# aelmiger/LINE-MOD-Pipeline

Hardware: AMD Instinct MI355X
Metric: detections/sec (higher is better)
Workload: dtype u8

## Files before the change

line-mod-pipeline_amd/build.py:

```python
import os
import subprocess
import sys

HERE = os.path.dirname(os.path.abspath(__file__))
CSRC = os.path.join(HERE, "csrc")
LIB_DIR = os.path.join(HERE, "lib")
LIB = os.path.join(LIB_DIR, "liblinemod_hip.so")
HIP_SOURCES = ["lm_k_preprocess.hip", "lm_k_mask.hip", "lm_k_scan.hip", "lm_k_refine.hip", "lm_k_post.hip", "lm_k_icp.hip", "lm_k_verify.hip", "lm_k_gen.hip", "lm_k_eval.hip",
               "lm_detector.hip", "lm_detector_upload.hip", "lm_detector_post.hip", "lm_detector_gather.hip", "lm_detector_io.hip", "lm_detector_debug.hip", "lm_detector_icp.hip", "lm_detector_gen.hip", "lm_detector_eval.hip", "lm_comm.hip"]
CXX_SOURCES = ["lm_host.cpp", "lm_extract.cpp", "lm_yaml.cpp"]
HEADERS = ["lm_common.h", "lm_kernels.h", "lm_dev.h", "lm_dev_color.h", "lm_dev_depth.h", "lm_dev_memories.h", "lm_detector_impl.h", "lm_host.h", "lm_extract.h", "lm_median25.h", "lm_yaml.h", "lm_comm.h",
           os.path.join("..", "..", "include", "linemod_hip.h")]
FLAGS = ["-O3", "-std=c++17", "-fPIC", "-ffp-contract=off", "-Wall", "-Wno-unused-function", "-Wno-unused-value"]
ARCH = "gfx950"


def _stale(target, deps):
    if not os.path.exists(target):
        return True
    t = os.path.getmtime(target)
    return any(os.path.exists(d) and os.path.getmtime(d) > t for d in deps)


def build(force=False, verbose=False):
    hipcc = os.environ.get("HIPCC", "/opt/rocm/bin/hipcc")
    os.makedirs(LIB_DIR, exist_ok=True)
    obj_dir = os.path.join(HERE, "build")
    os.makedirs(obj_dir, exist_ok=True)
    headers = [os.path.join(CSRC, h) for h in HEADERS]
    for h in headers:
        if not os.path.exists(h):
            raise FileNotFoundError("header missing from the checkout: " + h)
    objs, cmds = [], []
    for src in HIP_SOURCES + CXX_SOURCES:
        sp = os.path.join(CSRC, src)
        if not os.path.exists(sp):
            raise FileNotFoundError("source file missing from the checkout: " + sp)
        obj = os.path.join(obj_dir, src + ".o")
        objs.append(obj)
        if force or _stale(obj, [sp] + headers + [os.path.abspath(__file__)]):
            cmd = [hipcc] + FLAGS
            if src.endswith(".hip"):
                cmd += ["--offload-arch=" + ARCH]
            else:
                cmd += ["-x", "c++"]
            cmds.append(cmd + ["-c", sp, "-o", obj])
    if cmds:
        from concurrent.futures import ThreadPoolExecutor
        try:
            ncpu = len(os.sched_getaffinity(0))
        except AttributeError:
            ncpu = os.cpu_count() or 1
        jobs = max(1, min(len(cmds), int(os.environ.get("LM_BUILD_JOBS", "0")) or min(ncpu, 8)))

        def run(cmd):
            if verbose:
                print(" ".join(cmd), file=sys.stderr)
            subprocess.check_call(cmd)
        with ThreadPoolExecutor(max_workers=jobs) as ex:
            list(ex.map(run, cmds))
    if force or _stale(LIB, objs):
        cmd = [hipcc, "-shared", "-fPIC", "--offload-arch=" + ARCH, "-o", LIB] + objs + ["-lz", "-ldl"]
        if verbose:
            print(" ".join(cmd), file=sys.stderr)
        subprocess.check_call(cmd)
    return LIB


if __name__ == "__main__":
    print(build(force="--force" in sys.argv, verbose=True))
```

line-mod-pipeline_amd/csrc/lm_detector.hip:

```cpp
#include "lm_detector_impl.h"

namespace lmd {

thread_local std::string g_err;
int fail(int code, const std::string& msg) { g_err = msg; return code; }

bool any_lane_busy(const lm_detector* d) {
    for (const lm_detector::Lane& ln : d->lanes) if (ln.busy) return true;
    return false;
}

void free_device_bank(lm_detector* d) {
    hipFree(d->d_item_t); hipFree(d->d_item_chunk); hipFree(d->d_scan_off); hipFree(d->d_scan_P);
    hipFree(d->d_scan_n); hipFree(d->d_t_global); hipFree(d->d_t_class);
    hipFree(d->d_off1); hipFree(d->d_offn); hipFree(d->d_offs3); d->d_off1 = d->d_offn = d->d_offs3 = nullptr;
    hipFree(d->d_offl); hipFree(d->d_offsl); hipFree(d->d_litem); d->d_offl = d->d_offsl = d->d_litem = nullptr;
    for (auto& it : d->items1) { hipFree(it.d_t); hipFree(it.d_chunk); }
    d->items1.clear();
    d->d_item_t = d->d_item_chunk = d->d_scan_off = nullptr;
    d->d_scan_P = d->d_scan_n = d->d_t_global = d->d_t_class = nullptr;
    for (int l = 0; l < LM_MAX_LEVELS; ++l) {
        hipFree(d->d_ref_meta[l]); hipFree(d->d_ref_feat[l]);
        d->d_ref_meta[l] = nullptr; d->d_ref_feat[l] = nullptr;
    }
}


int ensure_device(lm_detector* d) {
    if (d->dev_ready) {
        HIP_TRY(hipSetDevice(d->cfg.device));
        return LM_OK;
    }
    int ndev = 0;
    hipError_t e = hipGetDeviceCount(&ndev);
    if (e != hipSuccess || ndev <= 0)
        return fail(LM_ERR_NO_DEVICE, "no HIP device available: liblinemod_hip has no CPU fallback");
    if (d->cfg.device < 0 || d->cfg.device >= ndev) return fail(LM_ERR_INVALID, "device ordinal out of range");
    HIP_TRY(hipSetDevice(d->cfg.device));
    d->scanl_lds = lmk_scanl_raise_lds();
    const lm_config& c = d->cfg;
    const int M = c.num_modalities, L = c.pyramid_levels, S = c.frame_slots;
    size_t off = 0;
    d->off_bgr[0] = off; off += (size_t)c.width * c.height * 3;
    d->off_depth = off; off += align_up((size_t)c.width * c.height * 2, 256);
    off = align_up(off, 256);
    for (int l = 1; l < L; ++l) { d->off_bgr[l] = off; off += align_up((size_t)d->lw[l] * d->lh[l] * 3, 256); }
    for (int l = 0; l < L; ++l)
        for (int m = 0; m < M; ++m) { d->off_quant[l][m] = off; off += align_up((size_t)d->lw[l] * d->lh[l], 256); }
    for (int l = 0; l < L; ++l) { d->off_lm[l] = off; off += align_up(d->geom[l].arena_bytes, 256); }
    d->off_cscratch = off; off += align_up(lmk_color_scratch_bytes(c.width, c.height), 256);
    d->off_cscratch1 = off; off += align_up(lmk_color_scratch_bytes(d->lw[L > 1 ? 1 : 0], d->lh[L > 1 ? 1 : 0]), 256);
    d->off_dscratch = off; off += align_up((size_t)c.width * c.height, 256);
    d->cmask_wpr = (c.width + 31) / 32;
    d->off_cmask = off; off += align_up((size_t)d->cmask_wpr * c.height * 4, 256);
    d->match_mask_pitch = align_up((size_t)c.width, 64);
    d->frame_stride = align_up(off, 4096);
    HIP_TRY(hipMalloc(reinterpret_cast<void**>(&d->frame_arena), d->frame_stride * S));
    HIP_TRY(hipMemset(d->frame_arena, 0, d->frame_stride * S));
    off = 0;
    d->off_hdr = off; off += 256;
    d->off_cand = off; off += align_up((size_t)d->max_cand * sizeof(LmCand), 256);
    d->off_keys = off; off += align_up((size_t)d->max_match * 16, 256);
    d->off_out = off; off += align_up((size_t)LM_SORT_CAP * sizeof(LmOutMatch), 256);
    d->aux_stride = align_up(off, 4096);
    HIP_TRY(hipMalloc(reinterpret_cast<void**>(&d->aux_arena), d->aux_stride * S));
    HIP_TRY(hipMemset(d->aux_arena, 0, d->aux_stride * S));
    d->host_stride = align_up(sizeof(LmHostBlock), 256);
    HIP_TRY(hipHostMalloc(reinterpret_cast<void**>(&d->host_blocks), d->host_stride * S, hipHostMallocMapped));
    std::memset(d->host_blocks, 0, d->host_stride * S);
    lm_detector::Lane& l0 = d->lanes[0];
    HIP_TRY(hipMalloc(reinterpret_cast<void**>(&l0.d_raw_thr), 128 * sizeof(int)));
    HIP_TRY(hipHostMalloc(reinterpret_cast<void**>(&l0.h_raw_thr), 128 * sizeof(int)));
    d->plan_stride_cap = std::max(S / 8, 1) + 8;
    const size_t plan_words = 24 * (size_t)d->plan_stride_cap + 16;
    HIP_TRY(hipMalloc(reinterpret_cast<void**>(&d->d_plan), LM_NLANES * plan_words * sizeof(u32)));
    for (int l = 0; l < LM_NLANES; ++l) d->lanes[l].plan = d->d_plan + (size_t)l * plan_words;
    HIP_TRY(hipStreamCreateWithFlags(&l0.stream, hipStreamNonBlocking));
    for (int l = 1; l < LM_NLANES; ++l) HIP_TRY(hipStreamCreateWithFlags(&d->lanes[l].stream, hipStreamNonBlocking));
    for (int k = 0; k < LM_NCOPY; ++k) {
        HIP_TRY(hipStreamCreateWithFlags(&d->copy_stream[k], hipStreamNonBlocking));
        d->up_seq_next[k] = 1; d->up_seq_done[k] = 0;
    }
    for (auto& ev : l0.ev) HIP_TRY(hipEventCreate(&ev));
    l0.created = true;
    d->slots.assign(S, Slot());
    for (Slot& s : d->slots) {
        HIP_TRY(hipEventCreateWithFlags(&s.ev_up, hipEventDisableTiming));
        HIP_TRY(hipEventCreateWithFlags(&s.ev_bgr, hipEventDisableTiming));
    }
    HIP_TRY(hipMalloc(reinterpret_cast<void**>(&d->d_resp_tab), 256 * sizeof(u64) + 256));
    HIP_TRY(hipMalloc(reinterpret_cast<void**>(&d->d_scan_stat), 4096 * sizeof(unsigned long long)));
    HIP_TRY(hipMemset(d->d_scan_stat, 0, 4096 * sizeof(unsigned long long)));
    HIP_TRY(hipMalloc(reinterpret_cast<void**>(&d->d_sim_lut), 256));
    HIP_TRY(hipMalloc(reinterpret_cast<void**>(&d->d_normal_lut), 2 * 8000 + 16));
    HIP_TRY(hipDeviceSynchronize());
    if (const char* ev = getenv("LM_REFINE_STAT")) {
        if (atoi(ev) > 0 && hipMalloc(reinterpret_cast<void**>(&d->d_refine_stat), 8 * sizeof(unsigned long long)) == hipSuccess)
            (void)hipMemset(d->d_refine_stat, 0, 8 * sizeof(unsigned long long));
    }
    d->dev_ready = true;
    d->luts_dirty = true;
    d->bank_dirty = true; d->hulls_dirty = true;
    return LM_OK;
}

int ensure_luts(lm_detector* d) {
    if (!d->luts_dirty) return LM_OK;
    u64 tab[256 + 32];
    u8* miss = reinterpret_cast<u8*>(tab + 256);
    int below4 = 0;
    for (int v = 0; v < 256; ++v) {
        u64 e = 0;
        miss[v] = 0;
        for (int o = 0; o < 8; ++o) {
            u8 r = std::max(d->sim_lut[32 * o + (v & 15)], d->sim_lut[32 * o + 16 + (v >> 4)]);
            e |= (u64)r << (8 * o);
            if (r < 4) { miss[v] |= (u8)(1u << o); below4 = std::max(below4, (int)r); }
        }
        tab[v] = e;
    }
    d->miss_delta = 4 - below4;
    HIP_TRY(hipDeviceSynchronize());
    HIP_TRY(hipMemcpy(d->d_resp_tab, tab, sizeof(tab), hipMemcpyHostToDevice));
    HIP_TRY(hipMemcpy(d->d_sim_lut, d->sim_lut, 256, hipMemcpyHostToDevice));
    {
        u8 both[2 * 8000 + 16] = {};
        std::memcpy(both, d->normal_lut, 8000);
        for (int i = 0; i < 8000; ++i) {
            const u8 v = d->normal_lut[i];
            const unsigned rank = v ? (unsigned)__builtin_ffs((int)v) : 0u;
            both[LMK_NORMAL_CODE_OFFSET + i] = (u8)(rank < 4 ? 8 * rank : (rank < 8 ? 8 * (rank - 4) + 4 : 32u));
        }
        HIP_TRY(hipMemcpy(d->d_normal_lut, both, sizeof(both), hipMemcpyHostToDevice));
    }
    d->luts_dirty = false;
    return LM_OK;
}

int ensure_bank(lm_detector* d) {
    if (!d->bank_dirty) return LM_OK;
    HIP_TRY(hipDeviceSynchronize());
    free_device_bank(d);
    std::string err;
    if (!lmh::build_device_bank(d->bank, d->cfg, d->geom, d->hb, d->scan_list_order, err)) return fail(LM_ERR_INVALID, err);
    int rc;
    if ((rc = upload_vec(&d->d_item_t, d->hb.item_t))) return rc;
    if ((rc = upload_vec(&d->d_item_chunk, d->hb.item_chunk))) return rc;
    if ((rc = upload_vec(&d->d_scan_off, d->hb.scan_off))) return rc;
    if ((rc = upload_vec(&d->d_scan_P, d->hb.scan_P))) return rc;
    if ((rc = upload_vec(&d->d_scan_n, d->hb.scan_n))) return rc;
    if (d->hb.fpad1) {
        if ((rc = upload_vec(&d->d_off1, d->hb.off1))) return rc;
        if ((rc = upload_vec(&d->d_offn, d->hb.offn))) return rc;
        if ((rc = upload_vec(&d->d_offs3, d->hb.offs3))) return rc;
    }
    if (d->hb.lds_ok) {
        if ((rc = upload_vec(&d->d_offl, d->hb.offl))) return rc;
        if ((rc = upload_vec(&d->d_offsl, d->hb.offsl))) return rc;
        if ((rc = upload_vec(&d->d_litem, d->hb.lrec))) return rc;
    }
    if ((rc = upload_vec(&d->d_t_global, d->hb.t_global))) return rc;
    if ((rc = upload_vec(&d->d_t_class, d->hb.t_class))) return rc;
    for (int l = 0; l + 1 < d->cfg.pyramid_levels; ++l) {
        if ((rc = upload_vec(&d->d_ref_meta[l], d->hb.ref_meta[l]))) return rc;
        if ((rc = upload_vec(&d->d_ref_feat[l], d->hb.ref_feat[l]))) return rc;
    }
    d->bank_dirty = false;
    return LM_OK;
}

int check_slots(lm_detector* d, int first, int n) {
    if (first < 0 || n < 0 || first + n > (int)d->slots.size()) return fail(LM_ERR_INVALID, "slot out of range");
    return LM_OK;
}

bool normal_lut_onehot(lm_detector* d) {
    if (d->lut_onehot < 0) {
        d->lut_onehot = 1;
        for (int i = 0; i < 8000; ++i) { const u8 v = d->normal_lut[i]; if (v & (v - 1)) { d->lut_onehot = 0; break; } }
    }
    return d->lut_onehot != 0;
}

void enqueue_depth_pyramid(lm_detector* d, lm_detector::Lane& ln, int first, int n) {
    for (int l = 1; l < d->cfg.pyramid_levels; ++l)
        lmk_nn_half(ln.stream, d->quant(first, l - 1, 1), d->lw[l - 1], d->quant(first, l, 1), d->lw[l], d->lh[l],
                    d->frame_stride, n);
}

int refuse_checked_slots(const lm_detector* d, int first, int n) {
    if (d->cc_inflight && d->cc_pending && first <= d->cc_hi && d->cc_lo < first + n) return fail(LM_ERR_INVALID, "slot is read by a colour check in flight: call lm_color_check_end first");
    if (d->dc_inflight && d->dc_pending && first <= d->dc_hi && d->dc_lo < first + n) return fail(LM_ERR_INVALID, "slot is read by depth counts in flight: call lm_depth_counts_end first");
    const int icp_slot = d->icp_slot.load();
    if (icp_slot >= first && icp_slot < first + n) return fail(LM_ERR_INVALID, "slot is read by an ICP refinement in flight");
    return LM_OK;
}

lmh::ScanInputs scan_inputs(const lm_detector* d, const lm_detector::Lane& ln) {
    const LmLevelGeom& g = d->geom[d->cfg.pyramid_levels - 1];
    lmh::ScanInputs in;
    in.form = d->scan_form; in.M = d->cfg.num_modalities;
    in.nibble = g.nibble != 0; in.planes = g.plane_ori != 0; in.lds_fits = lmh::lds_image_fits(g, in.M);
    in.bank_built = !d->bank_dirty;
    in.scanl_bank = d->hb.lds_ok && d->d_litem; in.scanl_device = d->scanl_lds;
    in.fpad1 = d->hb.fpad1; in.items1_by_L = d->hb.items1_by_L; in.items4 = (long long)d->hb.item_t.size();
    in.frame_stride = d->frame_stride; in.arena_bytes = g.arena_bytes;
    in.threshold = ln.raw_thr_for; in.scan1_min_threshold = d->scan1_min_threshold;
    in.scanl_min_slots = d->scanl_min_slots; in.scanl_R = d->scanl_R;
    return in;
}

void enqueue_lm(lm_detector* d, lm_detector::Lane& ln, int first, int n, int l, int m, u32 planes) {
    hipStream_t st = ln.stream;
    const size_t fs = d->frame_stride;
    const LmLevelGeom& g = d->geom[l];
    const int sp = g.spread_only ? 1 : g.nibble ? 2 : 0;
    u8* dst = d->lm(first, l) + (size_t)m * g.mod_stride;
    if (m == 0 || l == 0)
        lmk_linear_memories(st, d->quant(first, l, m), g.w, 0, sp, g.w, g.h, g.T, d->d_resp_tab, dst, g.ori_stride, fs, fs, n, planes);
    else
        lmk_linear_memories(st, d->quant(first, l - 1, 1), d->lw[l - 1], 1, sp, g.w, g.h, g.T, d->d_resp_tab, dst,
                            g.ori_stride, fs, fs, n, planes);
}

int slot_weight(const lm_detector* d) {
    const long px = (long)d->lw[0] * d->lh[0];
    const int w = d->work_weight_by_pixels ? (int)(px / (640L * 480L)) : 1;
    return w < 1 ? 1 : w;
}

bool any_match_mask(const lm_detector* d, int first, int n) {
    for (int i = first; i < first + n; ++i)
        if (d->slots[i].match_mask_on[0] || d->slots[i].match_mask_on[1] || d->slots[i].rule_on) return true;
    return false;
}

int hsv_bound(double b) { return (int)std::lrint(std::min(256.0, std::max(-1.0, b))); }

int ensure_hsv_div(lm_detector* d) {
    if (d->d_hsv_div) return LM_OK;
    std::vector<int> tab(512, 0);
    for (int i = 1; i < 256; ++i) {
        tab[(size_t)i] = (int)std::lrint((255 << 12) / (1.0 * i));
        tab[256 + (size_t)i] = (int)std::lrint((180 << 12) / (6.0 * i));
    }
    int* p = nullptr;
    HIP_TRY(hipMalloc(reinterpret_cast<void**>(&p), tab.size() * sizeof(int)));
    hipStream_t st = d->lanes[0].stream;
    if (hipMemcpyAsync(p, tab.data(), tab.size() * sizeof(int), hipMemcpyHostToDevice, st) != hipSuccess ||
        hipStreamSynchronize(st) != hipSuccess) {
        (void)hipFree(p);
        return fail(LM_ERR_HIP, "upload of the HSV division tables failed");
    }
    d->d_hsv_div = p;
    return LM_OK;
}

int check_mask_rule(const lm_detector* d, const lm_mask_rule* r, LmRule* out) {
    const lm_config& c = d->cfg;
    if (r->modalities <= 0 || r->modalities >= (1 << c.num_modalities))
        return fail(LM_ERR_INVALID, "mask rule: modalities must name at least one modality the detector has (bit 0 colour, bit 1 depth)");
    if (r->use_depth && c.num_modalities < 2)
        return fail(LM_ERR_INVALID, "mask rule: a depth gate needs the depth frame, which a colour-only detector does not keep on the device");
    if (r->use_depth && (r->zmin < 0 || r->zmax > 65535 || r->zmin > r->zmax))
        return fail(LM_ERR_INVALID, "mask rule: depth gate needs 0 <= zmin <= zmax <= 65535");
    if (r->grow < 0 || r->grow > LM_RULE_MAX_GROW) return fail(LM_ERR_INVALID, "mask rule: grow out of range (0 .. 16)");
    const lm_rect& q = r->rect;
    const bool no_rect = q.width == 0 && q.height == 0;
    if (!no_rect && (q.x < 0 || q.y < 0 || q.width <= 0 || q.height <= 0 || q.x > c.width - q.width || q.y > c.height - q.height))
        return fail(LM_ERR_INVALID, "mask rule: the rectangle must lie inside the frame");
    if (!lmk_mask_rule_fits(c.width)) return fail(LM_ERR_INVALID, "mask rule: frame too wide for the rule kernel");
    LmRule o{};
    o.use_depth = r->use_depth != 0; o.keep_invalid = r->keep_invalid != 0; o.use_hsv = r->use_hsv != 0;
    o.zmin = r->zmin; o.zmax = r->zmax; o.grow = r->grow;
    for (int k = 0; k < 3; ++k) { o.hsv.lo[k] = hsv_bound(r->lower[k]); o.hsv.hi[k] = hsv_bound(r->upper[k]); }
    o.rx = no_rect ? 0 : q.x; o.ry = no_rect ? 0 : q.y; o.rw = no_rect ? c.width : q.width; o.rh = no_rect ? c.height : q.height;
    *out = o;
    return LM_OK;
}

void enqueue_mask_rules(lm_detector* d, lm_detector::Lane& ln, int first, int n) {
    const lm_config& c = d->cfg;
    LmRuleArgs a{};
    a.bgr = d->bgr(0, 0); a.depth = c.num_modalities == 2 ? d->depth(0) : nullptr; a.slot_stride = d->frame_stride;
    a.divtab = d->d_hsv_div; a.w = c.width; a.h = c.height; a.mask_pitch = (u32)d->match_mask_pitch;
    int kinds = 0;
    for (int i = first; i < first + n; ++i) {
        const Slot& s = d->slots[i];
        if (!s.rule_on) continue;
        int k = 0;
        while (k < kinds && std::memcmp(&a.rule[k], &s.rule_dev, sizeof(LmRule)) != 0) ++k;
        if (k == LM_RULE_KINDS) { lmk_mask_rule(ln.stream, a); a.n = 0; kinds = 0; k = 0; }
        if (k == kinds) a.rule[kinds++] = s.rule_dev;
        a.slot[a.n] = (u16)i; a.kind[a.n] = (u8)k; a.plane[a.n] = s.d_rule_mask;
        if (++a.n == LM_MASK_SLOTS) { lmk_mask_rule(ln.stream, a); a.n = 0; kinds = 0; }
    }
    lmk_mask_rule(ln.stream, a);
}

static_assert(LM_MAX_LEVELS <= LM_MASK_LEVELS, "LmMaskArgs holds LM_MASK_LEVELS levels");
void enqueue_match_masks(lm_detector* d, lm_detector::Lane& ln, int first, int n) {
    const lm_config& c = d->cfg;
    LmMaskArgs a{};
    a.frame = d->frame_arena; a.slot_stride = d->frame_stride;
    a.levels = c.pyramid_levels; a.mask_pitch = (u32)d->match_mask_pitch;
    a.vec_rows = 1;
    for (int l = 0; l < c.pyramid_levels; ++l) {
        for (int m = 0; m < c.num_modalities; ++m) a.off_quant[l][m] = (u32)d->off_quant[l][m];
        a.w[l] = (u32)d->lw[l];
        a.vec_begin[l + 1] = a.vec_begin[l] + (u32)((size_t)d->lw[l] * d->lh[l] / 16);
        if (d->lw[l] % 16) a.vec_rows = 0;
    }
    a.vec_depth = a.vec_begin[1];
    for (int i = first; i < first + n; ++i) {
        const Slot& s = d->slots[i];
        if (!s.match_mask_on[0] && !(c.num_modalities == 2 && s.match_mask_on[1])) continue;
        a.slot[a.n] = (u16)i;
        a.cmask[a.n] = s.match_mask_on[0] ? s.d_match_mask : nullptr;
        a.dmask[a.n] = (c.num_modalities == 2 && s.match_mask_on[1]) ? s.d_match_mask + d->match_mask_pitch * c.height : nullptr;
        if (++a.n == LM_MASK_SLOTS) { lmk_match_mask(ln.stream, a); a.n = 0; }
    }
    if (a.n) lmk_match_mask(ln.stream, a);
    a.n = 0;
    for (int i = first; i < first + n; ++i) {
        const Slot& s = d->slots[i];
        if (!s.rule_on) continue;
        a.slot[a.n] = (u16)i;
        a.cmask[a.n] = (s.rule.modalities & 1) ? s.d_rule_mask : nullptr;
        a.dmask[a.n] = (c.num_modalities == 2 && (s.rule.modalities & 2)) ? s.d_rule_mask : nullptr;
        if (++a.n == LM_MASK_SLOTS) { lmk_match_mask(ln.stream, a); a.n = 0; }
    }
    if (a.n) lmk_match_mask(ln.stream, a);
}

void enqueue_preprocess(lm_detector* d, lm_detector::Lane& ln, int first, int n) {
    const lm_config& c = d->cfg;
    const int M = c.num_modalities, L = c.pyramid_levels;
    const lmh::Layout layout = lmh::plan_layout(scan_inputs(d, ln), n);
    for (int i = 0; i < n; ++i) d->slots[first + i].layout = layout;
    const u32 planes = layout == lmh::Layout::Responses ? 0u : d->geom[L - 1].plane_ori | (layout == lmh::Layout::SpreadAndPlanes ? 0x80000000u : 0u);
    const size_t fs = d->frame_stride;
    const int weight = slot_weight(d);
    struct WeightGuard { explicit WeightGuard(int w) { lmk_set_slot_weight(w); } ~WeightGuard() { lmk_set_slot_weight(1); } } weight_guard(weight);
    const int n_eff = n * weight;
    const bool few = n_eff <= d->phase_max_slots;
    bool others_busy = false;
    for (int o = 0; o < LM_NLANES; ++o) others_busy |= (&d->lanes[o] != &ln && d->lanes[o].busy);
    const bool fuse_batch = d->batch_phases == 1 || (d->batch_phases == 2 && !others_busy);
    const bool masked = any_match_mask(d, first, n);
    if (!masked && (few || (fuse_batch && n_eff >= 16)) && L == 2) {
        LmPhaseArgs pa{};
        pa.bgr0 = d->bgr(first, 0); pa.bgr1 = d->bgr(first, 1); pa.depth = M == 2 ? d->depth(first) : nullptr;
        pa.cs0 = d->cscratch(first, 0); pa.cs1 = d->cscratch(first, 1); pa.ds = d->dscratch(first);
        pa.qc0 = d->quant(first, 0, 0); pa.qc1 = d->quant(first, 1, 0); pa.qd0 = M == 2 ? d->quant(first, 0, 1) : nullptr;
        pa.lm_c0 = d->lm(first, 0); pa.lm_c1 = d->lm(first, 1);
        pa.lm_d0 = d->lm(first, 0) + d->geom[0].mod_stride; pa.lm_d1 = d->lm(first, 1) + d->geom[1].mod_stride;
        pa.w = d->lw[0]; pa.h = d->lh[0];
        pa.weak_threshold = c.weak_threshold; pa.dist_thr = c.distance_threshold; pa.diff_thr = c.difference_threshold;
        pa.normal_lut = d->d_normal_lut; pa.resp_tab = d->d_resp_tab; pa.ori_stride1 = d->geom[1].ori_stride; pa.plane_ori1 = planes;
        pa.slot_stride = fs; pa.nslots = n;
        auto mode = [&](int l) { return d->geom[l].spread_only ? 1 : d->geom[l].nibble ? 2 : 0; };
        const bool onehot = M == 2 ? normal_lut_onehot(d) : true;
        if (M <= 2 && d->lw[1] * 2 == d->lw[0] && d->lh[1] * 2 == d->lh[0]) {
            if (few && lmk_phases_supported(pa, d->geom[0].T, d->geom[1].T, mode(0), mode(1), onehot)) {
                lmk_preprocess_phases(ln.stream, pa, d->geom[0].T);
                return;
            }
            if (!few && lmk_batch_phases_supported(pa, d->geom[0].T, d->geom[1].T, mode(0), mode(1), onehot)) {
                lmk_preprocess_batch_phases(ln.stream, pa, d->geom[0].T);
                return;
            }
        }
    }
    const bool blur_pyr = L >= 2 && lmk_blur_pyrdown(ln.stream, d->bgr(first, 0), d->lw[0], d->lh[0], d->cscratch(first, 0), d->bgr(first, 1),
                                                      d->quant(first, 0, 0), fs, n);
    bool grads_done = false;
    if (L == 2 && blur_pyr && d->lw[1] * 2 == d->lw[0] && d->lh[1] * 2 == d->lh[0] && lmk_cgrad_levels_wanted(d->lw[0], d->lh[0], n) &&
        lmk_color_blur(ln.stream, d->bgr(first, 1), d->lw[1], d->lh[1], d->cscratch(first, 1), fs, n)) {
        grads_done = lmk_cgrad_levels(ln.stream, d->cscratch(first, 0), d->lw[0], d->lh[0], d->quant(first, 0, 0), d->cscratch(first, 1), d->lw[1], d->lh[1],
                                      d->quant(first, 1, 0), c.weak_threshold, fs, n);
        if (!grads_done)
            for (int l = 0; l < L; ++l) lmk_color_quantize(ln.stream, d->bgr(first, l), d->lw[l], d->lh[l], c.weak_threshold, d->quant(first, l, 0), nullptr, d->cscratch(first, l), fs, n, true);
        grads_done = true;
    }
    for (int l = 0; l < L; ++l) {
        if (l > 0 && !(l == 1 && blur_pyr)) lmk_pyrdown(ln.stream, d->bgr(first, l - 1), d->lw[l - 1], d->lh[l - 1], d->bgr(first, l), fs, n);
        if (!grads_done)
        lmk_color_quantize(ln.stream, d->bgr(first, l), d->lw[l], d->lh[l], c.weak_threshold, d->quant(first, l, 0),
                           nullptr, d->cscratch(first, l), fs, n, l == 0 && blur_pyr);
        if (M == 2 && l == 0)
            lmk_depth_quantize(ln.stream, d->depth(first), d->lw[0], d->lh[0], c.distance_threshold,
                               c.difference_threshold, d->d_normal_lut, normal_lut_onehot(d), d->quant(first, 0, 1),
                               d->dscratch(first), fs, n);
    }
    if (masked) {
        enqueue_mask_rules(d, ln, first, n);
        enqueue_match_masks(d, ln, first, n);
    }
    if (M == 2 && L > 2) enqueue_depth_pyramid(d, ln, first, n);
    for (int l = 0; l < L; ++l)
        for (int m = 0; m < M; ++m) enqueue_lm(d, ln, first, n, l, m, l == L - 1 ? planes : 0u);
}

void fill_raw_thr(int* tab, float threshold) {
    for (int n = 0; n < 128; ++n) tab[n] = static_cast<int>(2 * n + (threshold / 100.f) * (2 * n) + 0.5f);
}

int item_range(lm_detector* d, int class_idx, ItemRange* r) {
    const int nc = (int)d->bank.classes.size();
    if (class_idx >= nc || class_idx < -1) return fail(LM_ERR_INVALID, "class index out of range");
    if (class_idx < 0) { r->lo = 0; r->n = (int)d->hb.item_t.size(); r->t_lo = 0; r->t_hi = (int)d->hb.t_global.size(); }
    else {
        r->lo = d->hb.class_item_lo[class_idx]; r->n = d->hb.class_item_hi[class_idx] - r->lo;
        r->t_lo = d->hb.class_t_lo[class_idx]; r->t_hi = d->hb.class_t_hi[class_idx];
    }
    return LM_OK;
}

int item_ranges(lm_detector* d, std::vector<int>& classes, std::vector<ItemRange>& out) {
    const int nc = (int)d->bank.classes.size();
    out.clear();
    for (int c : classes) if (c < -1 || c >= nc) return fail(LM_ERR_INVALID, "class index out of range");
    std::sort(classes.begin(), classes.end());
    classes.erase(std::unique(classes.begin(), classes.end()), classes.end());
    if (classes.empty() || classes[0] < 0) {
        if (classes.size() > 1) return fail(LM_ERR_INVALID, "class index -1 (all classes) cannot be combined with others");
        classes.assign(1, -1);
        out.push_back(ItemRange{0, (int)d->hb.item_t.size(), 0, (int)d->hb.t_global.size()});
        return LM_OK;
    }
    for (int c : classes) {
        const int lo = d->hb.class_item_lo[c], hi = d->hb.class_item_hi[c];
        if (!out.empty() && out.back().lo + out.back().n == lo && out.back().t_hi == d->hb.class_t_lo[c]) { out.back().n += hi - lo; out.back().t_hi = d->hb.class_t_hi[c]; }
        else out.push_back(ItemRange{lo, hi - lo, d->hb.class_t_lo[c], d->hb.class_t_hi[c]});
// ... 842 lines not shown
```

line-mod-pipeline_amd/csrc/lm_dev_depth.h:

```cpp
#pragma once
#include "lm_dev.h"
#include "lm_median25.h"

namespace {

#define DT_W 64
#define DT_H 8
#define N_W (DT_W + 4)
#define N_H (DT_H + 4)
#define D_W (DT_W + 14)
#define D_H (DT_H + 14)
#define D_PITCH 80
#define D_LOADS ((D_H * D_W + 255) / 256)

typedef unsigned short us2 __attribute__((ext_vector_type(2)));
#define LM_CE(a, b) { us2 t_ = __builtin_elementwise_min(a, b); b = __builtin_elementwise_max(a, b); a = t_; }

__global__ __launch_bounds__(256) void k_depth_quantize(const u16* __restrict__ depth0, int w, int h, int dist_thr,
                                                         int diff_thr, const u8* __restrict__ lut,
                                                         u8* __restrict__ quant0, size_t slot_stride) {
    __shared__ u16 dt[D_H][D_PITCH];
    __shared__ u8 nt[N_H][N_W + 4];
    const u16* depth = slot_ptr(depth0, slot_stride);
    u8* quant = slot_ptr(quant0, slot_stride);
    const int tid = threadIdx.x;
    const int ox = blockIdx.x * DT_W, oy = blockIdx.y * DT_H;
    {
        u16 v[D_LOADS];
#pragma unroll
        for (int k = 0; k < D_LOADS; ++k) {
            int i = tid + k * 256;
            int r = i / D_W, c = i - r * D_W;
            int gy = oy - 7 + r, gx = ox - 7 + c;
            v[k] = (i < D_H * D_W && gy >= 0 && gy < h && gx >= 0 && gx < w) ? depth[(size_t)gy * w + gx] : (u16)0;
        }
#pragma unroll
        for (int k = 0; k < D_LOADS; ++k) {
            int i = tid + k * 256;
            if (i < D_H * D_W) { int r = i / D_W; dt[r][i - r * D_W] = v[k]; }
        }
    }
    __syncthreads();
    for (int i = tid; i < N_H * N_W; i += 256) {
        int ty = i / N_W, tx = i - ty * N_W;
        int gy = clampi(oy - 2 + ty, 0, h - 1), gx = clampi(ox - 2 + tx, 0, w - 1);
        u8 out = 0;
        if (gy >= 5 && gy < h - 6 && gx >= 5 && gx < w - 6) {
            const int ly = gy - (oy - 7), lx = gx - (ox - 7);
            int d = dt[ly][lx];
            if (d < dist_thr) {
                int A0 = 0, A1 = 0, A3 = 0, b0 = 0, b1 = 0;
#pragma unroll
                for (int jj = -1; jj <= 1; ++jj)
#pragma unroll
                    for (int ii = -1; ii <= 1; ++ii) {
                        if (ii == 0 && jj == 0) continue;
                        int di = ii * 5, dj = jj * 5;
                        int delta = (int)dt[ly + dj][lx + di] - d;
                        int ad = delta < 0 ? -delta : delta;
                        int f = ad < diff_thr ? 1 : 0;
                        int fi = f * di, fj = f * dj;
                        A0 += fi * di; A1 += fi * dj; A3 += fj * dj;
                        b0 += fi * delta; b1 += fj * delta;
                    }
                int det = A0 * A3 - A1 * A1;
                int ddx = A3 * b0 - A1 * b1;
                int ddy = -A1 * b0 + A0 * b1;
                float nx = (float)(1150LL * ddx);
                float ny = (float)(1150LL * ddy);
                float nz = (float)(-(long long)det * d);
                float len = __fsqrt_rn(__fadd_rn(__fadd_rn(__fmul_rn(nx, nx), __fmul_rn(ny, ny)), __fmul_rn(nz, nz)));
                if (len > 0) {
                    float inv = __fdiv_rn(1.0f, len);
                    nx = __fmul_rn(nx, inv); ny = __fmul_rn(ny, inv); nz = __fmul_rn(nz, inv);
                    int v1 = (int)__fadd_rn(__fmul_rn(nx, 10.f), 10.f);
                    int v2 = (int)__fadd_rn(__fmul_rn(ny, 10.f), 10.f);
                    int v3 = (int)__fadd_rn(__fmul_rn(nz, 20.f), 20.f);
                    int flat = v3 * 400 + v2 * 20 + v1;
                    out = (flat >= 0 && flat < 8000) ? lut[flat] : 0;
                }
            }
        }
        nt[ty][tx] = out;
    }
    __syncthreads();
    {
        const int ty = tid >> 5, tx = (tid & 31) * 2;
        const int gy = oy + ty, gx = ox + tx;
        us2 v[25];
#pragma unroll
        for (int j = 0; j < 5; ++j) {
            unsigned short b[6];
#pragma unroll
            for (int ii = 0; ii < 6; ++ii) b[ii] = nt[ty + j][tx + ii];
#pragma unroll
            for (int ii = 0; ii < 5; ++ii) { us2 p; p[0] = b[ii]; p[1] = b[ii + 1]; v[j * 5 + ii] = p; }
        }
        LM_MEDIAN25_NETWORK(v)
        const us2 med = v[LM_MEDIAN25_OUT];
        if (gy < h) {
            if (gx < w) quant[(size_t)gy * w + gx] = (u8)med[0];
            if (gx + 1 < w) quant[(size_t)gy * w + gx + 1] = (u8)med[1];
        }
    }
}

__device__ __forceinline__ u32 pk_sub_u16_sat(u32 a, u32 b) {
    u32 r;
    asm("v_pk_sub_u16 %0, %1, %2 clamp" : "=v"(r) : "v"(a), "v"(b));
    return r;
}
__device__ __forceinline__ u32 pk_min_u16(u32 a, u32 b) {
    u32 r;
    asm("v_pk_min_u16 %0, %1, %2" : "=v"(r) : "v"(a), "v"(b));
    return r;
}
__device__ __forceinline__ u32 pk_mul_lo_u16(u32 a, u32 b) {
    u32 r;
    asm("v_pk_mul_lo_u16 %0, %1, %2" : "=v"(r) : "v"(a), "v"(b));
    return r;
}
__device__ __forceinline__ u32 pk_sub_i16_op(u32 a, u32 b) {
    u32 r;
    asm("v_pk_sub_i16 %0, %1, %2" : "=v"(r) : "v"(a), "v"(b));
    return r;
}
__device__ __forceinline__ u32 pk_add_i16_op(u32 a, u32 b) {
    u32 r;
    asm("v_pk_add_i16 %0, %1, %2" : "=v"(r) : "v"(a), "v"(b));
    return r;
}
template <bool HI>
__device__ __forceinline__ int mad_i16h(u32 a, u32 b, int c) {
    int r;
    if (HI) asm("v_mad_i32_i16 %0, %1, %2, %3 op_sel:[1,1,0,0]" : "=v"(r) : "v"(a), "v"(b), "v"(c));
    else asm("v_mad_i32_i16 %0, %1, %2, %3" : "=v"(r) : "v"(a), "v"(b), "v"(c));
    return r;
}
__device__ __forceinline__ u32 hw_u16(const u32x4* A, int hw) {
    const u32 d = A[hw >> 3][(hw >> 1) & 3];
    return (hw & 1) ? (d >> 16) : (d & 0xFFFFu);
}

__device__ __forceinline__ float dn_rcp7(float d) {
    const float r0 = __builtin_amdgcn_rcpf(d);
    const float e = __builtin_fmaf(-d, r0, 1.0f);
    const float r1 = __builtin_fmaf(e, r0, r0);
    const float err0 = __builtin_fmaf(-d, r1, 1.0f);
    const float q1 = __builtin_fmaf(err0, r1, r1);
    const float err1 = __builtin_fmaf(-d, q1, 1.0f);
    return __builtin_fmaf(err1, r1, q1);
}
__device__ __forceinline__ float dn_sqrt_bare(float x) { return __builtin_amdgcn_sqrtf(x); }
__device__ __forceinline__ float dn_sqrt9(float x) {
    const float s = __builtin_amdgcn_sqrtf(x);
    const float s_dn = __builtin_bit_cast(float, __builtin_bit_cast(u32, s) - 1u);
    const float s_up = __builtin_bit_cast(float, __builtin_bit_cast(u32, s) + 1u);
    const float r_dn = __builtin_fmaf(-s_dn, s, x);
    const float r_up = __builtin_fmaf(-s_up, s, x);
    float r = r_dn <= 0.0f ? s_dn : s;
    return r_up > 0.0f ? s_up : r;
}
__device__ __forceinline__ float dn_rcp3(float d) {
    const float r0 = __builtin_amdgcn_rcpf(d);
    const float e = __builtin_fmaf(-d, r0, 1.0f);
    return __builtin_fmaf(e, r0, r0);
}
__device__ __forceinline__ float dn_sqrt5(float x) {
    const float y = __builtin_amdgcn_rsqf(x);
    const float g = __fmul_rn(x, y), hf = __fmul_rn(0.5f, y);
    const float e = __builtin_fmaf(-g, g, x);
    return __builtin_fmaf(e, hf, g);
}
__device__ __forceinline__ float dn_sqrt4(float x) {
    const float s = __builtin_amdgcn_sqrtf(x), y = __builtin_amdgcn_rsqf(x);
    const float e = __builtin_fmaf(-s, s, x);
    return __builtin_fmaf(e, __fmul_rn(0.5f, y), s);
}
__device__ __forceinline__ float dn_inv_from_rsq(float x, float len) {
    const float y = __builtin_amdgcn_rsqf(x);
    const float e = __builtin_fmaf(-len, y, 1.0f);
    return __builtin_fmaf(e, y, y);
}
__device__ __forceinline__ float dn_rcp(float d) { return dn_rcp3(d); }
__device__ __forceinline__ float dn_sqrt(float x) { return dn_sqrt5(x); }
template <bool SMALL, bool QUOT = false>
__device__ __forceinline__ u32 dn_label(int det, int ddx, int ddy, int d, bool ok, const u8* __restrict__ lut) {
    if (QUOT) { det = mul_i24(det, 625); if (!SMALL) { ddx = mul_i24(ddx, 125); ddy = mul_i24(ddy, 125); } }
    float nx = SMALL ? (float)(QUOT ? mul_i24(ddx, 143750) : ddx * 1150) : (float)((double)ddx * 1150.0);
    float ny = SMALL ? (float)(QUOT ? mul_i24(ddy, 143750) : ddy * 1150) : (float)((double)ddy * 1150.0);
    float nz = (float)(-mul_i24(det, d));
    const float len0 = dn_sqrt(__fadd_rn(__fadd_rn(__fmul_rn(nx, nx), __fmul_rn(ny, ny)), __fmul_rn(nz, nz)));
    const float len = len0 > 0.0f ? len0 : 1.0f;
    const float inv = dn_rcp(len);
    nx = __fmul_rn(nx, inv); ny = __fmul_rn(ny, inv); nz = __fmul_rn(nz, inv);
    const int v1 = (int)__fadd_rn(__fmul_rn(nx, 10.f), 10.f);
    const int v2 = (int)__fadd_rn(__fmul_rn(ny, 10.f), 10.f);
    const int v3 = (int)__fadd_rn(__fmul_rn(nz, 20.f), 20.f);
    const u32 flat = (u32)mad_i24(v3, 400, mad_i24(v2, 20, v1));
    const u32 ecode = lut[LMK_NORMAL_CODE_OFFSET + min(flat, 8000u)];
    return ok ? ecode : 0u;
}

typedef float f32x2 __attribute__((ext_vector_type(2)));
template <bool SMALL>
__device__ __forceinline__ void dn_label2(int det0, int ddx0, int ddy0, int d0, bool ok0, int det1, int ddx1, int ddy1, int d1, bool ok1,
                                          const __amdgpu_buffer_rsrc_t lut_rsrc, u32& e0, u32& e1) {
    det0 = mul_i24(det0, 625); det1 = mul_i24(det1, 625);
    if (!SMALL) { ddx0 = mul_i24(ddx0, 125); ddy0 = mul_i24(ddy0, 125); ddx1 = mul_i24(ddx1, 125); ddy1 = mul_i24(ddy1, 125); }
    f32x2 nx, ny, nz;
    nx[0] = SMALL ? (float)mul_i24(ddx0, 143750) : (float)((double)ddx0 * 1150.0);
    nx[1] = SMALL ? (float)mul_i24(ddx1, 143750) : (float)((double)ddx1 * 1150.0);
    ny[0] = SMALL ? (float)mul_i24(ddy0, 143750) : (float)((double)ddy0 * 1150.0);
    ny[1] = SMALL ? (float)mul_i24(ddy1, 143750) : (float)((double)ddy1 * 1150.0);
    nz[0] = (float)(-mul_i24(det0, d0)); nz[1] = (float)(-mul_i24(det1, d1));
    const f32x2 sq = (nx * nx + ny * ny) + nz * nz;
    f32x2 y; y[0] = __builtin_amdgcn_rsqf(sq[0]); y[1] = __builtin_amdgcn_rsqf(sq[1]);
    const f32x2 g = sq * y, hf = y * 0.5f;
    const f32x2 len0 = __builtin_elementwise_fma(__builtin_elementwise_fma(-g, g, sq), hf, g);
    f32x2 len; len[0] = len0[0] > 0.0f ? len0[0] : 1.0f; len[1] = len0[1] > 0.0f ? len0[1] : 1.0f;
    f32x2 r0; r0[0] = __builtin_amdgcn_rcpf(len[0]); r0[1] = __builtin_amdgcn_rcpf(len[1]);
    const f32x2 inv = __builtin_elementwise_fma(__builtin_elementwise_fma(-len, r0, (f32x2)(1.0f)), r0, r0);
    nx = nx * inv; ny = ny * inv; nz = nz * inv;
    const f32x2 t1 = nx * 10.f + 10.f, t2 = ny * 10.f + 10.f, t3 = nz * 20.f + 20.f;
    const u32 flat0 = (u32)mad_i24((int)t3[0], 400, mad_i24((int)t2[0], 20, (int)t1[0]));
    const u32 flat1 = (u32)mad_i24((int)t3[1], 400, mad_i24((int)t2[1], 20, (int)t1[1]));
    const u32 c0 = (u32)__builtin_amdgcn_raw_buffer_load_b8(lut_rsrc, (int)(LMK_NORMAL_CODE_OFFSET + min(flat0, 8000u)), 0, 0);
    const u32 c1 = (u32)__builtin_amdgcn_raw_buffer_load_b8(lut_rsrc, (int)(LMK_NORMAL_CODE_OFFSET + min(flat1, 8000u)), 0, 0);
    e0 = ok0 ? c0 : 0u; e1 = ok1 ? c1 : 0u;
}

__global__ __launch_bounds__(256) void k_selftest_float_tail(unsigned long long* __restrict__ out) {
    const u32 lo = 0x3F800000u, hi_rcp = (127u + 42u) << 23, hi_sqrt = (127u + 84u) << 23;
    unsigned long long bad_rcp = 0, bad_sqrt = 0, bad_bare = 0, c_rcp7 = 0, c_sqrt9 = 0, c_sqrt4 = 0, c_inv = 0;
    for (u32 b = lo + blockIdx.x * 256u + threadIdx.x; b <= hi_sqrt; b += gridDim.x * 256u) {
        const float x = __builtin_bit_cast(float, b);
        if (b <= hi_rcp) bad_rcp += __builtin_bit_cast(u32, dn_rcp(x)) != __builtin_bit_cast(u32, __fdiv_rn(1.0f, x));
        const u32 want = __builtin_bit_cast(u32, __builtin_sqrtf(x));
        bad_sqrt += __builtin_bit_cast(u32, dn_sqrt(x)) != want;
        bad_bare += __builtin_bit_cast(u32, dn_sqrt_bare(x)) != want;
        if (b <= hi_rcp) c_rcp7 += __builtin_bit_cast(u32, dn_rcp7(x)) != __builtin_bit_cast(u32, __fdiv_rn(1.0f, x));
        c_sqrt9 += __builtin_bit_cast(u32, dn_sqrt9(x)) != want;
        c_sqrt4 += __builtin_bit_cast(u32, dn_sqrt4(x)) != want;
        c_inv += __builtin_bit_cast(u32, dn_inv_from_rsq(x, dn_sqrt(x))) != __builtin_bit_cast(u32, __fdiv_rn(1.0f, __builtin_sqrtf(x)));
    }
    if (blockIdx.x == 0 && threadIdx.x == 0) bad_sqrt += dn_sqrt(0.0f) > 0.0f ? 1u : 0u;
    if (bad_rcp) atomicAdd(&out[0], bad_rcp);
    if (bad_sqrt) atomicAdd(&out[1], bad_sqrt);
    if (bad_bare) atomicAdd(&out[2], bad_bare);
    if (c_rcp7) atomicAdd(&out[3], c_rcp7);
    if (c_sqrt9) atomicAdd(&out[4], c_sqrt9);
    if (c_sqrt4) atomicAdd(&out[5], c_sqrt4);
    if (c_inv) atomicAdd(&out[6], c_inv);
}

template <bool SMALL>
__device__ __forceinline__ void d_dnormal_t(const u32 vblock, const u16* __restrict__ depth0, int w, int h, int dist_thr, int diff_thr,
                                                  const u8* __restrict__ lut, u8* __restrict__ code0, size_t in_stride,
                                                  size_t tmp_stride, int gblocks, int nslots) {
    u32 slot, tile;
    xcd_slot_tile_b(vblock, (u32)gblocks, (u32)nslots, slot, tile);
    const u16* depth = slot_ptr_s(depth0, in_stride, slot);
    u8* code = slot_ptr_s(code0, tmp_stride, slot);
    const int ng = w >> 3;
    const int gid = (int)(tile * 256u) + (int)threadIdx.x;
    const int y = gid / ng, g = gid - y * ng;
    if (y >= h) return;
    u32 out[2] = {0, 0};
    if (y >= 5 && y < h - 6) {
        u32x4 R[3][3];
#pragma unroll
        for (int j = 0; j < 3; ++j) {
            const u8* row = reinterpret_cast<const u8*>(depth + (size_t)(y + 5 * (j - 1)) * w) + 16 * g - 16;
#pragma unroll
            for (int k = 0; k < 3; ++k) {
                const bool ok = !(k == 0 && g == 0) && !(k == 2 && g == ng - 1);
                R[j][k] = ok ? ld16(row + 16 * k) : u32x4{0, 0, 0, 0};
            }
        }
        if (diff_thr >= 0 && diff_thr <= 5461) {
            const __amdgpu_buffer_rsrc_t lut_rsrc = __builtin_amdgcn_make_buffer_rsrc(const_cast<u8*>(lut), 0, 2 * 8000 + 16, 0x00020000);
            u32 D[3][12];
#pragma unroll
            for (int j = 0; j < 3; ++j)
#pragma unroll
                for (int k = 0; k < 12; ++k) D[j][k] = R[j][k >> 2][k & 3];
            const u32 THR = (u32)diff_thr * 0x00010001u;
#pragma unroll
            for (int k = 0; k < 4; ++k) {
                const u32 C = D[1][4 + k];
                u32 F[3][3], G[3][3];
#pragma unroll
                for (int jj = -1; jj <= 1; ++jj)
#pragma unroll
                    for (int ii = -1; ii <= 1; ++ii) {
                        if (ii == 0 && jj == 0) continue;
                        const u32* Dr = D[jj + 1];
                        const u32 N = ii == 0 ? Dr[4 + k]
                                    : ii > 0 ? __builtin_amdgcn_alignbit(Dr[7 + k], Dr[6 + k], 16)
                                             : __builtin_amdgcn_alignbit(Dr[2 + k], Dr[1 + k], 16);
                        const u32 up = pk_sub_u16_sat(N, C), dn = pk_sub_u16_sat(C, N);
                        const u32 f = pk_min_u16(pk_sub_u16_sat(THR, up | dn), 0x00010001u);
                        F[jj + 1][ii + 1] = f;
                        G[jj + 1][ii + 1] = pk_mul_lo_u16(pk_sub_i16(up, dn), f);
                    }
                const u32 fdp = F[2][2] + F[0][0], fdm = F[2][0] + F[0][2];
                const u32 cd = fdp + fdm;
                const u32 cx = pk_sub_i16(fdp, fdm);
                const u32 ci = F[1][2] + F[1][0] + cd, cj = F[2][1] + F[0][1] + cd;
                const u32 ga = pk_sub_i16(G[2][2], G[0][0]), gb = pk_sub_i16(G[0][2], G[2][0]);
                const u32 sx = pk_add_i16(pk_add_i16(pk_sub_i16(G[1][2], G[1][0]), ga), gb);
                const u32 sy = pk_sub_i16(pk_add_i16(pk_sub_i16(G[2][1], G[0][1]), ga), gb);
                const u32 ncx = pk_sub_i16(0u, cx);
                const int d0 = (int)(C & 0xFFFFu), d1 = (int)(C >> 16);
                const int detq0 = mad_i16h<false>(ci, cj, mad_i16h<false>(ncx, cx, 0)), detq1 = mad_i16h<true>(ci, cj, mad_i16h<true>(ncx, cx, 0));
                const int ddxq0 = mad_i16h<false>(cj, sx, mad_i16h<false>(ncx, sy, 0)), ddxq1 = mad_i16h<true>(cj, sx, mad_i16h<true>(ncx, sy, 0));
                const int ddyq0 = mad_i16h<false>(ci, sy, mad_i16h<false>(ncx, sx, 0)), ddyq1 = mad_i16h<true>(ci, sy, mad_i16h<true>(ncx, sx, 0));
                u32 e0, e1;
                dn_label2<SMALL>(detq0, ddxq0, ddyq0, d0, d0 < dist_thr, detq1, ddxq1, ddyq1, d1, d1 < dist_thr, lut_rsrc, e0, e1);
                out[k >> 1] |= (e0 | (e1 << 8)) << (16 * (k & 1));
            }
        } else {
#pragma unroll
        for (int p = 0; p < 8; ++p) {
            const int d = (int)hw_u16(R[1], 8 + p);
            const bool valid = d < dist_thr;
            int ci = 0, cj = 0, cx = 0, sx = 0, sy = 0;
#pragma unroll
            for (int jj = -1; jj <= 1; ++jj)
#pragma unroll
                for (int ii = -1; ii <= 1; ++ii) {
                    if (ii == 0 && jj == 0) continue;
                    const int delta = (int)hw_u16(R[jj + 1], 8 + p + 5 * ii) - d;
                    const int ad = delta < 0 ? -delta : delta;
                    const int f = ad < diff_thr ? 1 : 0;
                    const int fd = ad < diff_thr ? delta : 0;
                    if (ii != 0) { ci += f; sx += ii * fd; }
                    if (jj != 0) { cj += f; sy += jj * fd; }
                    if (ii != 0 && jj != 0) cx += ii * jj * f;
                }
            const int A0 = 25 * ci, A3 = 25 * cj, A1 = 25 * cx, b0 = 5 * sx, b1 = 5 * sy;
            const int det = mul_i24(A0, A3) - mul_i24(A1, A1);
            const int ddx = mul_i24(A3, b0) - mul_i24(A1, b1);
            const int ddy = mul_i24(A0, b1) - mul_i24(A1, b0);
            const u32 e = dn_label<false>(det, ddx, ddy, d, valid, lut);
            out[p >> 2] |= e << (8 * (p & 3));
        }
        }
    }
    {
        const int xlo = 5 - 8 * g, xhi = (w - 6) - 8 * g;
        unsigned long long m = ~0ull;
        if (xlo > 0) m &= xlo >= 8 ? 0ull : (~0ull << (8 * xlo));
        if (xhi < 8) m &= xhi <= 0 ? 0ull : (~0ull >> (8 * (8 - xhi)));
        out[0] &= (u32)m; out[1] &= (u32)(m >> 32);
    }
    *reinterpret_cast<u32x2*>(code + (size_t)y * w + 8 * g) = u32x2{out[0], out[1]};
}
__device__ __forceinline__ void d_dnormal(const u32 vblock, const u16* __restrict__ depth0, int w, int h, int dist_thr, int diff_thr,
                                          const u8* __restrict__ lut, u8* __restrict__ code0, size_t in_stride,
                                          size_t tmp_stride, int gblocks, int nslots) {
    if (diff_thr >= 0 && diff_thr <= 249) d_dnormal_t<true>(vblock, depth0, w, h, dist_thr, diff_thr, lut, code0, in_stride, tmp_stride, gblocks, nslots);
    else d_dnormal_t<false>(vblock, depth0, w, h, dist_thr, diff_thr, lut, code0, in_stride, tmp_stride, gblocks, nslots);
}
__global__ __launch_bounds__(256) void k_dnormal(const u16* __restrict__ depth0, int w, int h, int dist_thr, int diff_thr,
                                                  const u8* __restrict__ lut, u8* __restrict__ code0, size_t in_stride,
                                                  size_t tmp_stride, int gblocks, int nslots) {
    d_dnormal(blockIdx.x, depth0, w, h, dist_thr, diff_thr, lut, code0, in_stride, tmp_stride, gblocks, nslots);
}

#define DM_ROWS 4
#ifndef DM_ROWS_BATCH
#define DM_ROWS_BATCH 16
#endif
template <int ROWS>
__device__ __forceinline__ void d_dmedian(const u32 vblock, const u8* __restrict__ code0, int w, int h, u8* __restrict__ quant0,
                                                  size_t tmp_stride, size_t out_stride, int gblocks, int nslots) {
    u32 slot, tile;
    xcd_slot_tile_b(vblock, (u32)gblocks, (u32)nslots, slot, tile);
    const u8* code = slot_ptr_s(code0, tmp_stride, slot);
    u8* quant = slot_ptr_s(quant0, out_stride, slot);
    const int ng = w >> 3;
    const int gid = (int)(tile * 256u) + (int)threadIdx.x;
    const int band = gid / ng, g = gid - band * ng;
    const int y0 = band * ROWS;
    if (y0 >= h) return;
    u32 ringE[5][8], ringO[5][8];
    u32 sumE[8] = {0, 0, 0, 0, 0, 0, 0, 0}, sumO[8] = {0, 0, 0, 0, 0, 0, 0, 0};
#pragma unroll
    for (int i = 0; i < ROWS + 4; ++i) {
        const int yy = clampi(y0 - 2 + i, 0, h - 1);
        const u32 ro = (u32)yy * (u32)w + 8u * (u32)g;
        const u8* row = code + ro;
        const u32x2 c = *reinterpret_cast<const u32x2*>(row);
        u32 e[12];
#pragma unroll
        for (int k = 0; k < 8; ++k) e[2 + k] = (c[k >> 2] >> (8 * (k & 3))) & 0xFFu;
        const u32 l = *reinterpret_cast<const u32*>(code + (g > 0 ? ro - 4u : ro)), r = *reinterpret_cast<const u32*>(code + (g + 1 < ng ? ro + 8u : ro + 4u));
        e[0] = g > 0 ? (l >> 16) & 0xFFu : e[2]; e[1] = g > 0 ? l >> 24 : e[2];
        e[10] = g + 1 < ng ? r & 0xFFu : e[9]; e[11] = g + 1 < ng ? (r >> 8) & 0xFFu : e[9];
        u32 oh[12];
#pragma unroll
        for (int k = 0; k < 12; ++k) oh[k] = (1u << (e[k] & 31u)) & ~(e[k] >> 5);
        u32 t3[10];
#pragma unroll
        for (int k = 0; k < 10; ++k) t3[k] = oh[k] + oh[k + 1] + oh[k + 2];
#pragma unroll
        for (int k = 0; k < 8; ++k) {
            const u32 hs = t3[k] + oh[k + 3] + oh[k + 4];
            const u32 E = hs & 0x0F0F0F0Fu, O = (hs >> 4) & 0x0F0F0F0Fu;
            if (i >= 5) { sumE[k] -= ringE[i % 5][k]; sumO[k] -= ringO[i % 5][k]; }
            ringE[i % 5][k] = E; ringO[i % 5][k] = O;
            sumE[k] += E; sumO[k] += O;
        }
        if (i >= 4) {
            const int y = y0 + i - 4;
            if (y < h) {
                u32 o[2] = {0, 0};
#pragma unroll
                for (int k = 0; k < 8; ++k) {
                    const u32 e1 = sumE[k] + (sumE[k] << 8), PE = e1 + (e1 << 16);
                    const u32 o0 = sumO[k] + (PE >> 24);
                    const u32 o1 = o0 + (o0 << 8), PO = o1 + (o1 << 16);
                    const u32 mE = (PE + 0x73737373u) & 0x80808080u;
                    const u32 mO = (PO + 0x73737373u) & 0x80808080u;
                    const u32 res = 128u >> (u32)(__builtin_popcount(mE) + __builtin_popcount(mO));
                    o[k >> 2] |= res << (8 * (k & 3));
                }
                *reinterpret_cast<u32x2*>(quant + ((u32)y * (u32)w + 8u * (u32)g)) = u32x2{o[0], o[1]};
            }
        }
    }
}
template <int ROWS>
__global__ __launch_bounds__(256) void k_dmedian(const u8* __restrict__ code0, int w, int h, u8* __restrict__ quant0,
                                                  size_t tmp_stride, size_t out_stride, int gblocks, int nslots) {
    d_dmedian<ROWS>(blockIdx.x, code0, w, h, quant0, tmp_stride, out_stride, gblocks, nslots);
}


}
```

Before: 198,400.

## Re-encode depth median counts as nibble prefix words to cut ALU work

Changes the normal-code encoding so each code maps to a cumulative nibble word (0x11111111 >> code), turning per-bin histograms into prefix counts directly. The 5x5 median then sums five ring rows and checks the threshold with a biased nibble-wise average trick, instead of keeping separate even/odd running sums and doing two prefix scans per pixel. This removes the sum/subtract bookkeeping and the prefix shifts in the depth median kernel, at the cost of re-adding five ring rows per output and depending on a new code-table layout.

```diff
diff --git a/line-mod-pipeline_amd/build.py b/line-mod-pipeline_amd/build.py
--- a/line-mod-pipeline_amd/build.py
+++ b/line-mod-pipeline_amd/build.py
@@ -9,7 +9,7 @@
 HIP_SOURCES = ["lm_k_preprocess.hip", "lm_k_mask.hip", "lm_k_scan.hip", "lm_k_refine.hip", "lm_k_post.hip", "lm_k_icp.hip", "lm_k_verify.hip", "lm_k_gen.hip", "lm_k_eval.hip",
                "lm_detector.hip", "lm_detector_upload.hip", "lm_detector_post.hip", "lm_detector_gather.hip", "lm_detector_io.hip", "lm_detector_debug.hip", "lm_detector_icp.hip", "lm_detector_gen.hip", "lm_detector_eval.hip", "lm_comm.hip"]
 CXX_SOURCES = ["lm_host.cpp", "lm_extract.cpp", "lm_yaml.cpp"]
-HEADERS = ["lm_common.h", "lm_kernels.h", "lm_dev.h", "lm_dev_color.h", "lm_dev_depth.h", "lm_dev_memories.h", "lm_detector_impl.h", "lm_host.h", "lm_extract.h", "lm_median25.h", "lm_yaml.h", "lm_comm.h",
+HEADERS = ["lm_common.h", "lm_kernels.h", "lm_dev.h", "lm_dev_color.h", "lm_dev_depth.h", "lm_dev_memories.h", "lm_detector_impl.h", "lm_host.h", "lm_extract.h", "lm_median25.h", "lm_median_counts.h", "lm_yaml.h", "lm_comm.h",
            os.path.join("..", "..", "include", "linemod_hip.h")]
 FLAGS = ["-O3", "-std=c++17", "-fPIC", "-ffp-contract=off", "-Wall", "-Wno-unused-function", "-Wno-unused-value"]
 ARCH = "gfx950"
diff --git a/line-mod-pipeline_amd/csrc/lm_detector.hip b/line-mod-pipeline_amd/csrc/lm_detector.hip
--- a/line-mod-pipeline_amd/csrc/lm_detector.hip
+++ b/line-mod-pipeline_amd/csrc/lm_detector.hip
@@ -1,4 +1,5 @@
 #include "lm_detector_impl.h"
+#include "lm_median_counts.h"
 
 namespace lmd {
 
@@ -129,7 +130,7 @@
         for (int i = 0; i < 8000; ++i) {
             const u8 v = d->normal_lut[i];
             const unsigned rank = v ? (unsigned)__builtin_ffs((int)v) : 0u;
-            both[LMK_NORMAL_CODE_OFFSET + i] = (u8)(rank < 4 ? 8 * rank : (rank < 8 ? 8 * (rank - 4) + 4 : 32u));
+            both[LMK_NORMAL_CODE_OFFSET + i] = (u8)lm_mc_rank_code(rank);
         }
         HIP_TRY(hipMemcpy(d->d_normal_lut, both, sizeof(both), hipMemcpyHostToDevice));
     }
diff --git a/line-mod-pipeline_amd/csrc/lm_dev_depth.h b/line-mod-pipeline_amd/csrc/lm_dev_depth.h
--- a/line-mod-pipeline_amd/csrc/lm_dev_depth.h
+++ b/line-mod-pipeline_amd/csrc/lm_dev_depth.h
@@ -1,6 +1,7 @@
 #pragma once
 #include "lm_dev.h"
 #include "lm_median25.h"
+#include "lm_median_counts.h"
 
 namespace {
 
@@ -385,8 +386,7 @@
     const int band = gid / ng, g = gid - band * ng;
     const int y0 = band * ROWS;
     if (y0 >= h) return;
-    u32 ringE[5][8], ringO[5][8];
-    u32 sumE[8] = {0, 0, 0, 0, 0, 0, 0, 0}, sumO[8] = {0, 0, 0, 0, 0, 0, 0, 0};
+    u32 ring[5][8];
 #pragma unroll
     for (int i = 0; i < ROWS + 4; ++i) {
         const int yy = clampi(y0 - 2 + i, 0, h - 1);
@@ -399,33 +399,23 @@
         const u32 l = *reinterpret_cast<const u32*>(code + (g > 0 ? ro - 4u : ro)), r = *reinterpret_cast<const u32*>(code + (g + 1 < ng ? ro + 8u : ro + 4u));
         e[0] = g > 0 ? (l >> 16) & 0xFFu : e[2]; e[1] = g > 0 ? l >> 24 : e[2];
         e[10] = g + 1 < ng ? r & 0xFFu : e[9]; e[11] = g + 1 < ng ? (r >> 8) & 0xFFu : e[9];
-        u32 oh[12];
-#pragma unroll
-        for (int k = 0; k < 12; ++k) oh[k] = (1u << (e[k] & 31u)) & ~(e[k] >> 5);
+        u32 cw[12];
+#pragma unroll
+        for (int k = 0; k < 12; ++k) cw[k] = lm_mc_word(e[k]);
         u32 t3[10];
 #pragma unroll
-        for (int k = 0; k < 10; ++k) t3[k] = oh[k] + oh[k + 1] + oh[k + 2];
-#pragma unroll
-        for (int k = 0; k < 8; ++k) {
-            const u32 hs = t3[k] + oh[k + 3] + oh[k + 4];
-            const u32 E = hs & 0x0F0F0F0Fu, O = (hs >> 4) & 0x0F0F0F0Fu;
-            if (i >= 5) { sumE[k] -= ringE[i % 5][k]; sumO[k] -= ringO[i % 5][k]; }
-            ringE[i % 5][k] = E; ringO[i % 5][k] = O;
-            sumE[k] += E; sumO[k] += O;
-        }
+        for (int k = 0; k < 10; ++k) t3[k] = cw[k] + cw[k + 1] + cw[k + 2];
+#pragma unroll
+        for (int k = 0; k < 8; ++k) ring[i % 5][k] = t3[k] + cw[k + 3] + cw[k + 4];
         if (i >= 4) {
             const int y = y0 + i - 4;
             if (y < h) {
                 u32 o[2] = {0, 0};
 #pragma unroll
                 for (int k = 0; k < 8; ++k) {
-                    const u32 e1 = sumE[k] + (sumE[k] << 8), PE = e1 + (e1 << 16);
-                    const u32 o0 = sumO[k] + (PE >> 24);
-                    const u32 o1 = o0 + (o0 << 8), PO = o1 + (o1 << 16);
-                    const u32 mE = (PE + 0x73737373u) & 0x80808080u;
-                    const u32 mO = (PO + 0x73737373u) & 0x80808080u;
-                    const u32 res = 128u >> (u32)(__builtin_popcount(mE) + __builtin_popcount(mO));
-                    o[k >> 2] |= res << (8 * (k & 3));
+                    const u32 A = ring[(i + 1) % 5][k] + ring[(i + 2) % 5][k] + ring[(i + 3) % 5][k];
+                    const u32 B3 = ring[(i + 4) % 5][k] + ring[i % 5][k] + LM_MC_BIAS;
+                    o[k >> 2] |= lm_mc_label(lm_mc_flags_biased(A, B3)) << (8 * (k & 3));
                 }
                 *reinterpret_cast<u32x2*>(quant + ((u32)y * (u32)w + 8u * (u32)g)) = u32x2{o[0], o[1]};
             }
diff --git a/line-mod-pipeline_amd/csrc/lm_median_counts.h b/line-mod-pipeline_amd/csrc/lm_median_counts.h
--- /dev/null
+++ b/line-mod-pipeline_amd/csrc/lm_median_counts.h
@@ -0,0 +1,20 @@
+#pragma once
+#include <stdint.h>
+
+#if defined(__HIPCC__)
+#define LM_MC_FN __host__ __device__ __forceinline__
+#else
+#define LM_MC_FN inline
+#endif
+
+LM_MC_FN uint32_t lm_mc_rank_code(uint32_t rank) { return rank < 8u ? 4u * rank : 29u; }
+
+LM_MC_FN uint32_t lm_mc_word(uint32_t code) { return 0x11111111u >> (code & 31u); }
+
+#define LM_MC_BIAS 0x33333333u
+LM_MC_FN uint32_t lm_mc_flags_biased(uint32_t A, uint32_t B3) {
+    return ((A & B3) + (((A ^ B3) >> 1) & 0x77777777u)) & 0x88888888u;
+}
+LM_MC_FN uint32_t lm_mc_flags(uint32_t A, uint32_t B) { return lm_mc_flags_biased(A, B + LM_MC_BIAS); }
+
+LM_MC_FN uint32_t lm_mc_label(uint32_t flags) { return 128u >> (uint32_t)__builtin_popcount(flags); }
```

After: 202,300, median of 6. 1.02x the previous value.
